# RKWin93/E2E-MAPPO-for-MT-FJSP

Hardware: AMD Instinct MI355X
Metric: env-steps/sec (batched J6M6E2) (higher is better)
Workload: dtype f64 (environment) / f32 (encoder: f32 storage and accumulation; 128x128 products on the 16-bit matrix cores from split f32 operands, f32-accurate: DESIGN.md §4)

## Files before the change

__graft_entry__.py:

```python
#!/usr/bin/env python3
import os
import sys

ROOT = os.path.dirname(os.path.abspath(__file__))
if ROOT not in sys.path:
    sys.path.insert(0, ROOT)


def build() -> None:
    from importlib import import_module
    import mtfjsp_amd
    _build = import_module("e2e-mappo-for-mt-fjsp_amd._build")
    lib = _build.build(force=True, verbose=True)
    capi = import_module("e2e-mappo-for-mt-fjsp_amd.capi")
    capi.lib()
    print("variant:", _build.build_variant("funcs", ["-DMTFJSP_BODY_FUNCS=3"]))
    from oracle import env_oracle
    print("oracle:", env_oracle.build(force=True))
    print("built", lib)


def smoke() -> None:
    import numpy as np
    import torch
    from importlib import import_module
    import mtfjsp_amd
    assert torch.cuda.is_available(), "smoke() needs cuda:0"
    batch_env = import_module("e2e-mappo-for-mt-fjsp_amd.batch_env")
    inst = import_module("e2e-mappo-for-mt-fjsp_amd.instances")
    from oracle.env_oracle import OracleBatch
    J, M, E, B = 6, 6, 2, 8
    T = J * M
    t, p, tt, edge = inst.generate_instances(B, J, M, E, seed=0)
    import random
    random.seed(0)
    w3 = inst.random_weights(B)
    env = batch_env.DeviceBatchEnv(J, M, E, B, obs_dtype="f64")
    env.load_instances(t, p, tt, edge=edge)
    env.scaler_init()
    env.reset(w3)
    orc = OracleBatch(t, p, tt, edge)
    orc.scaler_init()
    orc.reset(w3)
    a = torch.zeros(B, dtype=torch.int32, device=env.device); m = torch.zeros_like(a); j = torch.zeros_like(a)
    for s in range(T):
        env.random_actions(7, s, a, m, j)
        env.step(a, m)
        info, raw, _ = orc.step(a.cpu().numpy(), m.cpu().numpy())
        cand, mask = orc.job_mask_update(j.cpu().numpy())
        o = orc.observe()
        assert np.array_equal(env.info.cpu().numpy(), info), f"step {s}: rewards differ"
        assert np.array_equal(env.tasks_fea.cpu().numpy(), o["tfea"]), f"step {s}: tasks_fea differ"
        assert np.array_equal(env.dense_adj().cpu().numpy(), o["adj"]), f"step {s}: adj differ"
        assert np.array_equal(env.m_fea2.cpu().numpy(), o["mfea2"])
        assert np.array_equal(env.candidate.cpu().numpy(), cand) and np.array_equal(env.job_mask.cpu().numpy(), mask)
    assert bool(env.info[:, 1].all())
    _smoke_encoder()
    print("smoke OK: HIP env == oracle on", B, "instances x", T, "steps")


def _smoke_encoder() -> None:
    try:
        from importlib import import_module
        enc = import_module("e2e-mappo-for-mt-fjsp_amd.encoder")
    except ImportError:
        return
    if hasattr(enc, "smoke"):
        enc.smoke()


if __name__ == "__main__":
    cmd = sys.argv[1] if len(sys.argv) > 1 else "build"
    {"build": build, "smoke": smoke}[cmd]()
```

e2e-mappo-for-mt-fjsp_amd/_build.py:

```python
import os
import shutil
import subprocess

PKG = os.path.dirname(os.path.abspath(__file__))
CSRC = os.path.join(PKG, "csrc")
LIB = os.path.join(PKG, "libmtfjsp.so")
SOURCES = ["mtfjsp_env.hip", "mtfjsp_encoder.hip", "mtfjsp_gin_res.hip", "mtfjsp_pdr.hip", "mtfjsp_lookahead.hip", "mtfjsp_beam.hip", "mtfjsp_group.hip", "mtfjsp_hostgen.cpp"]
FLAGS = ["--offload-arch=gfx950", "-O3", "-ffp-contract=off", "-fPIC", "-std=c++17", "-Wall"]
SOURCE_FLAGS = {"mtfjsp_env.hip": ["-mllvm", "-amdgpu-sched-strategy=max-ilp"], "mtfjsp_gin_res.hip": ["-mllvm", "-amdgpu-sched-strategy=max-ilp"]}
if os.environ.get("MTFJSP_NO_SOURCE_FLAGS"):
    SOURCE_FLAGS = {}
if os.environ.get("MTFJSP_SOURCE_FLAGS_JSON"):
    import json
    SOURCE_FLAGS = json.loads(os.environ["MTFJSP_SOURCE_FLAGS_JSON"])


def hipcc():
    for c in (os.environ.get("HIPCC"), shutil.which("hipcc"), "/opt/rocm/bin/hipcc"):
        if c and os.path.exists(c):
            return c
    raise RuntimeError("hipcc not found")


def needs_build():
    if not os.path.exists(LIB):
        return True
    t = os.path.getmtime(LIB)
    deps = [os.path.join(CSRC, s) for s in SOURCES if os.path.exists(os.path.join(CSRC, s))]
    deps.append(os.path.join(PKG, "..", "include", "mtfjsp.h"))
    deps += [os.path.join(CSRC, f) for f in os.listdir(CSRC) if f.endswith((".h", ".hpp"))]
    return any(os.path.getmtime(d) > t for d in deps)


def _compile_link(out, extra_flags, verbose=False):
    import concurrent.futures
    import tempfile
    srcs = [s for s in SOURCES if os.path.exists(os.path.join(CSRC, s))]
    with tempfile.TemporaryDirectory(prefix="mtfjsp_build_") as tmp:
        def one(src):
            obj = os.path.join(tmp, src + ".o")
            cmd = [hipcc()] + FLAGS + SOURCE_FLAGS.get(src, []) + list(extra_flags) + ["-c", os.path.join(CSRC, src), "-o", obj]
            if verbose:
                print(" ".join(cmd))
            subprocess.check_call(cmd)
            return obj
        with concurrent.futures.ThreadPoolExecutor(len(srcs)) as ex:
            objs = list(ex.map(one, srcs))
        cmd = [hipcc(), "--offload-arch=gfx950", "-shared", "-fPIC"] + objs + ["-o", out]
        if verbose:
            print(" ".join(cmd))
        subprocess.check_call(cmd)
    return out


def build(force=False, verbose=False):
    if not force and not needs_build():
        return LIB
    return _compile_link(LIB, [], verbose)


def build_variant(tag, extra_flags, verbose=False):
    out = os.path.join(PKG, f"libmtfjsp_{tag}.so")
    srcs = [os.path.join(CSRC, s) for s in SOURCES]
    import hashlib
    hsh = hashlib.sha256(" ".join(FLAGS + list(extra_flags) + [repr(sorted(SOURCE_FLAGS.items()))]).encode())
    for d in sorted(srcs + [os.path.join(CSRC, f) for f in os.listdir(CSRC) if f.endswith((".h", ".hpp"))] + [os.path.join(PKG, "..", "include", "mtfjsp.h")]):
        hsh.update(open(d, "rb").read())
    stamp = out + ".srchash"
    if os.path.exists(out) and os.path.exists(stamp) and open(stamp).read() == hsh.hexdigest() and not os.environ.get("MTFJSP_REBUILD_VARIANTS"):
        return out
    _compile_link(out, extra_flags, verbose)
    with open(stamp, "w") as f:
        f.write(hsh.hexdigest())
    return out


if __name__ == "__main__":
    print(build(force=True, verbose=True))
```

e2e-mappo-for-mt-fjsp_amd/csrc/mtfjsp_gin_resident.h:

```cpp
#ifndef GR_KERNEL
#ifndef MTFJSP_GIN_RESIDENT_H
#define MTFJSP_GIN_RESIDENT_H
#include <type_traits>
#include <utility>
#include "mtfjsp_gin_res_select.h"

#ifndef GR_ABL
#define GR_ABL 0
#endif
#ifndef GR_NRES
#define GR_NRES 16
#endif
#ifndef GR_VRES
#define GR_VRES 1
#endif
#define GR_RING 6
#define GR_NBAR 6
#ifndef GR_GRP
#define GR_GRP 2
#endif
#ifndef GR_LOOK
#define GR_LOOK 2
#endif
#define GR_ROWB 272
#define GR_PLANE (32 * GR_ROWB)
#define GR_TILE (2 * GR_PLANE)
#define GR_MAXWARM 10
#ifndef GR_FX_DROP
#define GR_FX_DROP 1
#endif
#ifndef GR_FX_TAIL
#define GR_FX_TAIL 1
#endif
#ifndef GR_FX_SETUP
#define GR_FX_SETUP 1
#endif
struct GrShapeAny { static constexpr bool FIXED = false; static constexpr int T = 0, J = 0, IPC = 0; };
template <int T_, int J_, int IPC_> struct GrShapeFixed {
    static constexpr bool FIXED = true; static constexpr int T = T_, J = J_, IPC = IPC_;
    static_assert(T_ >= GR_MINT && T_ <= GR_MAXT && IPC_ * T_ == GR_ROWS && IPC_ * J_ <= GR_MAXCAND && (IPC_ * 128) % 256 == 0, "fixed shape: full 576-row workgroups");
};
typedef GrShapeFixed<GIN_RES_FX_T, GIN_RES_FX_J, GIN_RES_FX_IPC> GrShapeHeadline;
constexpr int gr_left_at(int T, int h, int rt)
{
    int left = ((16 * h) / T + 1) * T - 16 * h;
    for (int i = 0; i < rt; i++) { left -= 32; if (left <= 0) left += T; if (left <= 0) left += T; }
    return left;
}
constexpr int gr_max_chunks(int T)
{
    int m = 0;
    for (int i = 0; i < 16; i++) { const int r0 = i * T, c = ((r0 + T - 1) >> 4) - (r0 >> 4) + 1; m = c > m ? c : m; }
    return m;
}

#ifndef GR_MIX
#define GR_MIX 2
#endif
#ifndef GR_SETTLE
#define GR_SETTLE 1
#endif
#ifndef GR_FOLD_DPP
#define GR_FOLD_DPP 1
#endif
#ifndef GR_STAT_ASM
#define GR_STAT_ASM 0
#endif
#ifndef GR_PK
#define GR_PK 1
#endif
typedef float f32x16 __attribute__((ext_vector_type(16)));
typedef _Float16 gr_h8 __attribute__((ext_vector_type(8)));
typedef _Float16 gr_h2 __attribute__((ext_vector_type(2)));

struct GinResArgs {
    int B, T, J, ipc;
    const void *tfea; int feat_f64;
    const int *ell_col; const float *ell_val;
    const void *Wx32[6];
    float wsinv[6];
    const float *gamma[6], *beta[6];
    unsigned long long *stats;
    unsigned long long *stats_next;
    int wexp[6];
    int ffrac[6];
    unsigned long long *bar;
    unsigned long long epoch;
    unsigned *fail;
    unsigned *range_flag;
    const int *candidate;
    float *pooled;
    float *cand_feat;
    float *h_nodes;
    float *zspill;
    double inv_rows;
    int barrier_only;
    unsigned expect_extra;
    unsigned long long *stamps;
    const void *warm[GR_MAXWARM];
    unsigned warm_lines[GR_MAXWARM];
    int nwarm;
};
#define GR_STATS_PART (6 * 8 * HD * 2)
#define GR_STATS_SET GR_STATS_PART
#ifdef GR_STAMP
#define GR_STAMP_AT(i) do { if (tid == 0 && A.stamps) { A.stamps[(size_t)blockIdx.x * 64 + (i)] = __builtin_amdgcn_s_memrealtime(); \
                                                         if ((i) <= 30) A.stamps[(size_t)blockIdx.x * 64 + 33 + (i)] = __builtin_amdgcn_s_memtime(); } } while (0)
#else
#define GR_STAMP_AT(i) do { } while (0)
#endif

#define GR_OFF_PLANES 0
#define GR_OFF_RING (2 * GR_TILE)
#define GR_RING_BYTES ((2 * GR_LOOK - 2) * GR_TILE > GR_RING * 32 * HD * 4 ? (2 * GR_LOOK - 2) * GR_TILE : GR_RING * 32 * HD * 4)
#define GR_OFF_ELLC (GR_OFF_RING + GR_RING_BYTES)
#define GR_OFF_ELLV0 (GR_OFF_ELLC + GR_ROWS * 4)
#define GR_OFF_ELLV1 (GR_OFF_ELLV0 + GR_ROWS * 4)
#define GR_OFF_BN (GR_OFF_ELLV1 + GR_ROWS * 4)
#define GR_OFF_CAND (GR_OFF_BN + 2 * HD * 4)
// ... 280 lines not shown
        if (GR_ABL & 4) return;
#pragma unroll
        for (int i = 0; i < 8; i++) stat2(i, a[2 * i], a[2 * i + 1]);
    };
    auto split2x4 = [&](f32x2 v01, f32x2 v23, uint2 &p0, uint2 &p1) __attribute__((always_inline)) {
        const gr_h2 a = __builtin_convertvector(v01, gr_h2), b = __builtin_convertvector(v23, gr_h2);
#if GR_MIX == 2
        const gr_h2 c = gr_rem16(v01, a), d = gr_rem16(v23, b);
#else
        const f32x2 r01 = gr_rem2(v01, a), r23 = gr_rem2(v23, b);
        const gr_h2 c = __builtin_convertvector(r01, gr_h2), d = __builtin_convertvector(r23, gr_h2);
#endif
        p0 = make_uint2(__builtin_bit_cast(unsigned, a), __builtin_bit_cast(unsigned, b));
        p1 = make_uint2(__builtin_bit_cast(unsigned, c), __builtin_bit_cast(unsigned, d));
    };
    auto stats_tile = [&](auto Tc) __attribute__((always_inline)) {
        constexpr int RT = decltype(Tc)::value;
        stats_all(GR_TILEVAL(RT));
    };
    auto fold_stats = [&]() __attribute__((always_inline)) {
        float *red = s_ring;
        float *mine = red + (wave * 64 + lane) * 36;
#pragma unroll
        for (int j = 0; j < 4; j++) {
            *reinterpret_cast<float4 *>(mine + 4 * j) = make_float4(ts[2 * j][0], ts[2 * j][1], ts[2 * j + 1][0], ts[2 * j + 1][1]);
            *reinterpret_cast<float4 *>(mine + 16 + 4 * j) = make_float4(tq[2 * j][0], tq[2 * j][1], tq[2 * j + 1][0], tq[2 * j + 1][1]);
        }
#pragma unroll
        for (int i = 0; i < 8; i++) { ts[i] = f32x2{0.f, 0.f}; tq[i] = f32x2{0.f, 0.f}; }
        LDS_BARRIER();
        const int col = tid >> 1, kind = tid & 1, cw = col & 31;
        const float *src = red + ((col >> 5) * 64 + 32 * ((cw >> 2) & 1)) * 36 + 4 * (cw >> 3) + (cw & 3) + 16 * kind;
        float s0 = 0.f, s1 = 0.f, s2 = 0.f, s3 = 0.f;
#pragma unroll
        for (int i = 0; i < 32; i += 4) { s0 += src[i * 36]; s1 += src[(i + 1) * 36]; s2 += src[(i + 2) * 36]; s3 += src[(i + 3) * 36]; }
        return (s0 + s1) + (s2 + s3);
    };
    auto fold_stats_dpp = [&]() __attribute__((always_inline)) {
        const bool b4 = (lane & 16) != 0, b3 = (lane & 8) != 0, b2 = (lane & 4) != 0, b1 = (lane & 2) != 0, b0 = (lane & 1) != 0;
        auto dpp = [&](float x, auto Ctrl) __attribute__((always_inline)) {
            return __builtin_bit_cast(float, __builtin_amdgcn_update_dpp(0, __builtin_bit_cast(int, x), decltype(Ctrl)::value, 0xF, 0xF, true));
        };
        float v16[16];
#pragma unroll
        for (int c = 0; c < 16; c++) {
            const float a = ts[c >> 1][c & 1], q_ = tq[c >> 1][c & 1];
            v16[c] = (b4 ? q_ : a) + __shfl_xor(b4 ? a : q_, 16);
        }
#pragma unroll
        for (int i = 0; i < 8; i++) { ts[i] = f32x2{0.f, 0.f}; tq[i] = f32x2{0.f, 0.f}; }
        float v8[8];
#pragma unroll
        for (int c = 0; c < 8; c++) v8[c] = (b3 ? v16[c + 8] : v16[c]) + dpp(b3 ? v16[c] : v16[c + 8], std::integral_constant<int, 0x140>{});
        float v4[4];
#pragma unroll
        for (int c = 0; c < 4; c++) v4[c] = (b2 ? v8[c + 4] : v8[c]) + dpp(b2 ? v8[c] : v8[c + 4], std::integral_constant<int, 0x141>{});
        float v2[2];
#pragma unroll
        for (int c = 0; c < 2; c++) v2[c] = (b1 ? v4[c + 2] : v4[c]) + dpp(b1 ? v4[c] : v4[c + 2], std::integral_constant<int, 0x4E>{});
        return (b0 ? v2[1] : v2[0]) + dpp(b0 ? v2[0] : v2[1], std::integral_constant<int, 0xB1>{});
    };
    unsigned char *const pl0 = s_planes, *const pl1 = s_planes + GR_TILE, *const plr = reinterpret_cast<unsigned char *>(s_ring);
    auto plane_buf = [&](int i) __attribute__((always_inline)) { return i == 0 ? pl0 : i == 1 ? pl1 : plr + (i - 2) * GR_TILE; };
    auto produce_quarter = [&](auto Tc, auto Gc, unsigned char *pbuf) __attribute__((always_inline)) {
        constexpr int rt = decltype(Tc)::value, g = decltype(Gc)::value;
        unsigned char *dst = pbuf + n * GR_ROWB + (32 * wave + 8 * g + 4 * h) * 2;
        const float *bn = bn_of(rt);
        const float4 s4 = *reinterpret_cast<const float4 *>(bn + 32 * wave + 8 * g + 4 * h);
        const float4 h4 = *reinterpret_cast<const float4 *>(bn + HD + 32 * wave + 8 * g + 4 * h);
        const f32x16 &a = GR_TILEVAL(rt);
        uint2 p0, p1;
        split2x4(f32x2{bn_relu_ss(a[4 * g], s4.x, h4.x), bn_relu_ss(a[4 * g + 1], s4.y, h4.y)},
                 f32x2{bn_relu_ss(a[4 * g + 2], s4.z, h4.z), bn_relu_ss(a[4 * g + 3], s4.w, h4.w)}, p0, p1);
        *reinterpret_cast<uint2 *>(dst) = p0;
        *reinterpret_cast<uint2 *>(dst + GR_PLANE) = p1;
    };
    auto produce_tile = [&](auto Tc, unsigned char *pbuf) __attribute__((always_inline)) {
        gr_static_for<4>([&](auto Gc) __attribute__((always_inline)) { produce_quarter(Tc, Gc, pbuf); });
        __builtin_amdgcn_sched_barrier(0);
    };
    const unsigned char *xa0 = s_planes + n * GR_ROWB + 16 * h;
#define GR_FENCE() __builtin_amdgcn_sched_barrier(0)
#define GR_PIN_V() do { } while (0)
    auto consume_tile = [&](auto Tc) __attribute__((always_inline)) {
        constexpr int RT = decltype(Tc)::value;
        constexpr int PT = RT + GR_LOOK;
        constexpr bool NEXT = (PT < GR_NT) && !(GR_ABL & 1);
        constexpr bool STATS = RT > 0 && (GR_VRES || RT - 1 < GR_NRES) && !(GR_ABL & 4);
        const unsigned char *xa = plane_buf(RT % (2 * GR_LOOK)) + n * GR_ROWB + 16 * h;
        unsigned char *pnext = plane_buf(PT % (2 * GR_LOOK));
        const float *bn = bn_of(PT);
        gr_h8 xf[2][2];
#pragma unroll
        for (int p = 0; p < 2; p++) xf[0][p] = *reinterpret_cast<const gr_h8 *>(xa + p * GR_PLANE);
        float4 s4 = make_float4(0.f, 0.f, 0.f, 0.f), h4 = s4;
        if constexpr (NEXT) {
            s4 = *reinterpret_cast<const float4 *>(bn + 32 * wave + 4 * h);
            h4 = *reinterpret_cast<const float4 *>(bn + HD + 32 * wave + 4 * h);
        }
        constexpr bool VT = GR_VRES && RT >= GR_NRES;
        f32x16 atmp;
        f32x16 &a = RT < GR_NRES ? acc[RT < GR_NRES ? RT : 0] : VT ? zs[RT >= GR_NRES ? (RT - GR_NRES) & 1 : 0] : atmp;
        if constexpr (RT + GR_LOOK + 1 >= GR_NRES && RT + GR_LOOK + 1 < GR_NT) zload(std::integral_constant<int, RT + GR_LOOK + 1 - GR_NRES>{});
        gr_static_for<4>([&](auto Pc) __attribute__((always_inline)) {
            constexpr int g = decltype(Pc)::value;
            const gr_h8 *x0 = xf[0], *x1 = xf[1];
            f32x2 v01 = {0.f, 0.f}, v23 = {0.f, 0.f}, e01 = v01, e23 = v01;
            gr_h2 p01 = {0, 0}, p23 = p01, q01 = p01, q23 = p01;
            unsigned char *dst = pnext + n * GR_ROWB + (32 * wave + 8 * g + 4 * h) * 2;
            const f32x16 &nx = GR_TILEVAL(PT < GR_NT ? PT : RT);
            const f32x16 &pv = GR_TILEVAL(RT > 0 ? RT - 1 : 0);
            auto M = [&](int ks, int wp, int xp) __attribute__((always_inline)) {
                if (GR_ABL & 2) return;
                if constexpr (VT) mfma_v(a, wf[wp][ks], (ks & 1) ? x1[xp] : x0[xp], ks == 0 && wp == 0 && xp == 1);
                else if (ks == 0 && wp == 0 && xp == 1)
                    a = __builtin_amdgcn_mfma_f32_32x32x16_f16(wf[wp][ks], x0[xp], f32x16{0.f, 0.f, 0.f, 0.f, 0.f, 0.f, 0.f, 0.f, 0.f, 0.f, 0.f, 0.f, 0.f, 0.f, 0.f, 0.f}, 0, 0, 0);
                else a = __builtin_amdgcn_mfma_f32_32x32x16_f16(wf[wp][ks], (ks & 1) ? x1[xp] : x0[xp], a, 0, 0, 0);
            };
            M(2 * g, 0, 1);
            xf[1][0] = *reinterpret_cast<const gr_h8 *>(xa + 32 * (2 * g + 1));
            if constexpr (NEXT) { v01 = gr_fma2(f32x2{nx[4 * g], nx[4 * g + 1]}, f32x2{s4.x, s4.y}, f32x2{h4.x, h4.y});
                                  v23 = gr_fma2(f32x2{nx[4 * g + 2], nx[4 * g + 3]}, f32x2{s4.z, s4.w}, f32x2{h4.z, h4.w}); }
            GR_FENCE();
            M(2 * g, 1, 0);
            xf[1][1] = *reinterpret_cast<const gr_h8 *>(xa + GR_PLANE + 32 * (2 * g + 1));
            if constexpr (NEXT) { v01 = __builtin_elementwise_max(v01, f32x2{0.f, 0.f}); v23 = __builtin_elementwise_max(v23, f32x2{0.f, 0.f}); }
            GR_FENCE();
            M(2 * g, 0, 0);
            if constexpr (NEXT) { p01 = __builtin_convertvector(v01, gr_h2); p23 = __builtin_convertvector(v23, gr_h2); }
            if constexpr (NEXT && g < 3) s4 = *reinterpret_cast<const float4 *>(bn + 32 * wave + 8 * (g + 1) + 4 * h);
            GR_FENCE();
            M(2 * g + 1, 0, 1);
            if constexpr (g < 3) xf[0][0] = *reinterpret_cast<const gr_h8 *>(xa + 32 * (2 * g + 2));
            if constexpr (NEXT && !GR_MIX) { e01 = __builtin_convertvector(p01, f32x2); e23 = __builtin_convertvector(p23, f32x2); }
            if constexpr (NEXT && g < 3) h4 = *reinterpret_cast<const float4 *>(bn + HD + 32 * wave + 8 * (g + 1) + 4 * h);
            GR_FENCE();
            M(2 * g + 1, 1, 0);
            if constexpr (g < 3) xf[0][1] = *reinterpret_cast<const gr_h8 *>(xa + GR_PLANE + 32 * (2 * g + 2));
            if constexpr (NEXT) { if constexpr (GR_MIX == 2) { q01 = gr_rem16(v01, p01); q23 = gr_rem16(v23, p23); }
                                  else if constexpr (GR_MIX == 1) { v01 = gr_rem2(v01, p01); v23 = gr_rem2(v23, p23); } else { v01 = gr_sub2(v01, e01); v23 = gr_sub2(v23, e23); }
                                  if (!(GR_ABL & 8)) *reinterpret_cast<uint2 *>(dst) = make_uint2(__builtin_bit_cast(unsigned, p01), __builtin_bit_cast(unsigned, p23));
                                  if constexpr (GR_MIX != 2) { q01 = __builtin_convertvector(v01, gr_h2); q23 = __builtin_convertvector(v23, gr_h2); } }
            GR_FENCE();
            M(2 * g + 1, 0, 0);
            if constexpr (NEXT) { if (!(GR_ABL & 8)) *reinterpret_cast<uint2 *>(dst + GR_PLANE) = make_uint2(__builtin_bit_cast(unsigned, q01), __builtin_bit_cast(unsigned, q23));
                                  else asm volatile("" :: "v"(p01), "v"(p23), "v"(q01), "v"(q23)); }
            if constexpr (STATS) { stat2(2 * g, pv[4 * g], pv[4 * g + 1]); stat2(2 * g + 1, pv[4 * g + 2], pv[4 * g + 3]); }
            GR_FENCE();
        });
        if constexpr (RT >= GR_NRES && !GR_VRES) {
            stats_all(a);
            zstore(std::integral_constant<int, RT - GR_NRES>{}, a);
            GR_FENCE();
        }
        if constexpr (!VT && GR_SETTLE) { asm volatile("s_nop 1"); GR_FENCE(); }
    };
    auto consume_tile0 = [&](auto Tc) __attribute__((always_inline)) {
        constexpr int RT = decltype(Tc)::value;
        const unsigned char *xa = xa0 + 32 * (RT & 7);
        bf16x8 x[3];
#pragma unroll
        for (int p = 0; p < 3; p++) x[p] = *reinterpret_cast<const bf16x8 *>(xa + p * GR_PLANE);
        f32x16 a = {0.f, 0.f, 0.f, 0.f, 0.f, 0.f, 0.f, 0.f, 0.f, 0.f, 0.f, 0.f, 0.f, 0.f, 0.f, 0.f};
        a = __builtin_amdgcn_mfma_f32_32x32x16_bf16(w0f[0], x[2], a, 0, 0, 0);
        a = __builtin_amdgcn_mfma_f32_32x32x16_bf16(w0f[2], x[0], a, 0, 0, 0);
        a = __builtin_amdgcn_mfma_f32_32x32x16_bf16(w0f[1], x[1], a, 0, 0, 0);
        a = __builtin_amdgcn_mfma_f32_32x32x16_bf16(w0f[0], x[1], a, 0, 0, 0);
        a = __builtin_amdgcn_mfma_f32_32x32x16_bf16(w0f[1], x[0], a, 0, 0, 0);
        a = __builtin_amdgcn_mfma_f32_32x32x16_bf16(w0f[0], x[0], a, 0, 0, 0);
        if constexpr (RT < GR_NRES) acc[RT] = a;
        else if constexpr (GR_VRES) zs[(RT - GR_NRES) & 1] = a;
        else {
            stats_all(a);
            zstore(std::integral_constant<int, RT - GR_NRES>{}, a);
        }
        if constexpr (RT > 0 && (GR_VRES || RT - 1 < GR_NRES)) stats_tile(std::integral_constant<int, RT - 1>{});
        __builtin_amdgcn_sched_barrier(0);
    };
    float *s_wtab = s_ring + 1024 + 4 * (2 * 32 * 36);
    static_assert(!(GR_FX_SETUP && GR_FOLD_DPP) || (1024 + 4 * (2 * 32 * 36)) * 4 >= (2 * GR_LOOK - 2) * GR_TILE, "s_wtab lies past the plane buffers in the ring area");
    unsigned warm_word = 0;
    int slot[GR_NT];
    auto final_setup_a = [&]() __attribute__((always_inline)) {
        int tid_s = tid;
        if constexpr (FXS) asm volatile("" : "+v"(tid_s));
        for (int i = tid_s; i < 17 * 16; i += 256) s_wtab[i] = (i & 15) < (i >> 4) ? 1.0f : 0.0f;
        if (A.nwarm > 0) {
            unsigned l = (blockIdx.x >> 3) * 256u + (unsigned)tid_s;
            const unsigned char *wp = reinterpret_cast<const unsigned char *>(A.warm[0]);
            bool found = false;
            for (int w = 0; w < A.nwarm; w++) {
                const unsigned nl = A.warm_lines[w];
                if (!found && l < nl) { wp = reinterpret_cast<const unsigned char *>(A.warm[w]) + (size_t)l * 128; found = true; }
                if (!found) l -= nl;
            }
            warm_word = *reinterpret_cast<const unsigned *>(wp);
        }
    };
    auto final_setup_b = [&]() __attribute__((always_inline)) {
#ifndef GR_KEEP_MASKS
        asm volatile("" : "+v"(n_l));
#endif
#pragma unroll
        for (int rt = 0; rt < GR_NT; rt++) slot[rt] = (GR_ABL & 32) ? -1 : s_rowcand[rt * 32 + n_l];
    };
    auto layer_boundary = [&](auto Kc) __attribute__((always_inline)) {
        constexpr int k = decltype(Kc)::value;
        GR_STAMP_AT(4 + 4 * k);
        if constexpr (GR_VRES && GR_NT > GR_NRES) {
            asm volatile("s_nop 15\n\ts_nop 15" ::: "memory");
            stats_all(zs[(GR_NT - 1 - GR_NRES) & 1]);
        }
#if GR_FOLD_DPP
        (void)fold_stats;
        const float colsum = fold_stats_dpp();
        int lane_b = lane;
        if constexpr (FXS && k == 5) asm volatile("" : "+v"(lane_b));
        const int n_b = lane_b & 31, h_b = lane_b >> 5;
        const int kind = n_b >> 4, scol = 32 * wave + 8 * ((n_b & 15) >> 2) + 4 * h_b + (n_b & 3);
        constexpr int PAIR = 16;
#else
        const float colsum = fold_stats();
        const int kind = tid & 1, scol = tid >> 1;
        constexpr int PAIR = 1;
#endif
        const int sidx = 2 * scol + kind;
        if (k == 1) GR_STAMP_AT(2);
        const unsigned grp = blockIdx.x & 7u;
        {
            float x = colsum;
            if (!(__builtin_fabsf(x) * (kind ? A.wsinv[k] * A.wsinv[k] : A.wsinv[k]) < __builtin_ldexpf(1.0f, 51 - A.ffrac[k]))) {
                if (A.range_flag && !timed_out) __hip_atomic_store(A.range_flag, 1u, __ATOMIC_RELAXED, __HIP_MEMORY_SCOPE_SYSTEM);
// ... 97 lines not shown
#ifndef GR_KEEP_MASKS
        if constexpr (FXD) asm volatile("" : "+v"(n_l));
        else asm volatile("" : "+s"(nrows_l), "+v"(n_l));
#endif
        if constexpr (layer != 3) {
            gr_static_for<GR_LOOK>([&](auto Ic) __attribute__((always_inline)) { produce_tile(Ic, plane_buf(decltype(Ic)::value)); });
            LDS_BARRIER();
            unsigned *cnt = s_cnt + (layer - 1) * (GR_NT / GR_GRP);
            gr_static_for<GR_NT>([&](auto Tc) __attribute__((always_inline)) {
                constexpr int RT = decltype(Tc)::value;
                constexpr int step = RT / GR_GRP, back = GR_LOOK / GR_GRP;
                if constexpr (GR_LOOK > GR_GRP && RT % GR_GRP == 0 && step >= back) {
                    while (__builtin_amdgcn_readfirstlane(__hip_atomic_load(&cnt[step - back], __ATOMIC_RELAXED, __HIP_MEMORY_SCOPE_WORKGROUP)) < 4u)
                        __builtin_amdgcn_s_sleep(1);
                    asm volatile("" ::: "memory");
                    __builtin_amdgcn_sched_barrier(0);
                }
                consume_tile(Tc);
                GR_PIN_V();
                if constexpr (RT % GR_GRP == GR_GRP - 1) {
                    if constexpr (GR_LOOK > GR_GRP) {
                        asm volatile("" ::: "memory");
                        if (lane == 0) __hip_atomic_fetch_add(&cnt[step], 1u, __ATOMIC_RELAXED, __HIP_MEMORY_SCOPE_WORKGROUP);
                    } else LDS_BARRIER();
                }
                __builtin_amdgcn_sched_barrier(0);
            });
            if constexpr (GR_LOOK > GR_GRP) LDS_BARRIER();
            static_assert(GR_NT % GR_GRP == 0 && GR_GRP >= 1 && (GR_LOOK == GR_GRP || GR_LOOK == 2 * GR_GRP) && GR_LOOK <= GR_NRES, "tile groups");
        } else {
            auto write_h = [&](auto Tc) __attribute__((always_inline)) {
                constexpr int rt = decltype(Tc)::value;
                float *base = s_ring + ((rt % GR_RING) * 32 + n) * HD;
                gr_static_for<4>([&](auto Gc) __attribute__((always_inline)) {
                    constexpr int g = decltype(Gc)::value;
                    const float *bn = bn_of(rt);
                    const float4 s4 = *reinterpret_cast<const float4 *>(bn + 32 * wave + 8 * g + 4 * h);
                    const float4 h4 = *reinterpret_cast<const float4 *>(bn + HD + 32 * wave + 8 * g + 4 * h);
                    const f32x16 &a = GR_TILEVAL(rt);
                    const int ch = (8 * wave + 2 * g + h) ^ (n & 7);
                    *reinterpret_cast<float4 *>(base + 4 * ch) = make_float4(bn_relu_ss(a[4 * g], s4.x, h4.x), bn_relu_ss(a[4 * g + 1], s4.y, h4.y),
                                                                             bn_relu_ss(a[4 * g + 2], s4.z, h4.z), bn_relu_ss(a[4 * g + 3], s4.w, h4.w));
                });
                __builtin_amdgcn_sched_barrier(0);
            };
            auto ring_row = [&](int R) __attribute__((always_inline)) {
                const int t = R >> 5;
                return ((t - GR_RING * ((t * 43) >> 8)) * 32 + (R & 31)) * HD;
            };
            struct AggRow { const float *po, *px, *py; float w0, w1, inv; int s0, s1, s2; };
            auto agg_row = [&](int RT) __attribute__((always_inline)) {
                AggRow r;
                const int row = RT * 32 + n_l;
                const unsigned cp = s_ellc[row];
                const unsigned r0 = cp & 0xffffu, r1 = cp >> 16;
                r.w0 = s_ellv0[row]; r.w1 = s_ellv1[row];
                const int deg = 1 + (r0 != 0xffffu) + (r1 != 0xffffu);
                r.inv = deg == 1 ? 1.0f : deg == 2 ? 0.5f : (1.0f / 3.0f);
                const int n0 = r0 != 0xffffu ? (int)r0 : row, n1 = r1 != 0xffffu ? (int)r1 : row;
                r.po = s_ring + ((RT % GR_RING) * 32 + n) * HD; r.px = s_ring + ring_row(n0); r.py = s_ring + ring_row(n1);
                r.s0 = n & 7; r.s1 = n0 & 7; r.s2 = n1 & 7;
                return r;
            };
            auto agg_quarter_standalone = [&](const AggRow &r, int g, unsigned char *dst) __attribute__((always_inline)) {
                const int chl = 8 * wave + 2 * g + h;
                const float4 o = *reinterpret_cast<const float4 *>(r.po + 4 * (chl ^ r.s0));
                const float4 x = *reinterpret_cast<const float4 *>(r.px + 4 * (chl ^ r.s1));
                const float4 y = *reinterpret_cast<const float4 *>(r.py + 4 * (chl ^ r.s2));
                const f32x2 W0 = {r.w0, r.w0}, W1 = {r.w1, r.w1}, IV = {r.inv, r.inv};
                const f32x2 v01 = gr_mul2(gr_fma2(W1, f32x2{y.x, y.y}, gr_fma2(W0, f32x2{x.x, x.y}, f32x2{o.x, o.y})), IV);
                const f32x2 v23 = gr_mul2(gr_fma2(W1, f32x2{y.z, y.w}, gr_fma2(W0, f32x2{x.z, x.w}, f32x2{o.z, o.w})), IV);
                uint2 p0, p1;
                split2x4(v01, v23, p0, p1);
                *reinterpret_cast<uint2 *>(dst + 16 * g) = p0;
                *reinterpret_cast<uint2 *>(dst + 16 * g + GR_PLANE) = p1;
            };
            auto consume_agg = [&](auto Tc) __attribute__((always_inline)) {
                constexpr int RT = decltype(Tc)::value;
                constexpr bool NEXT = RT + 1 < GR_NT && !(GR_ABL & 1);
                constexpr bool WH = RT + 4 < GR_NT && !(GR_ABL & 1);
                constexpr int WT = WH ? RT + 4 : RT;
                constexpr bool STATS = RT > 0 && (GR_VRES || RT - 1 < GR_NRES) && !(GR_ABL & 4);
                constexpr bool VT = GR_VRES && RT >= GR_NRES;
                const unsigned char *xa = xa0 + (RT & 1) * GR_TILE;
                gr_h8 xf[2][2];
#pragma unroll
                for (int p = 0; p < 2; p++) xf[0][p] = *reinterpret_cast<const gr_h8 *>(xa + p * GR_PLANE);
                AggRow r = agg_row(NEXT ? RT + 1 : RT);
                unsigned char *dst = s_planes + ((RT + 1) & 1) * GR_TILE + n * GR_ROWB + (32 * wave + 4 * h) * 2;
                const float *bnw = bn_of(WT);
                float *hbase = s_ring + ((WT % GR_RING) * 32 + n) * HD;
                float4 s4 = make_float4(0.f, 0.f, 0.f, 0.f), h4 = s4;
                if constexpr (WH) {
                    s4 = *reinterpret_cast<const float4 *>(bnw + 32 * wave + 4 * h);
                    h4 = *reinterpret_cast<const float4 *>(bnw + HD + 32 * wave + 4 * h);
                }
                f32x16 atmp;
                f32x16 &a = RT < GR_NRES ? acc[RT < GR_NRES ? RT : 0] : VT ? zs[RT >= GR_NRES ? (RT - GR_NRES) & 1 : 0] : atmp;
                if constexpr (RT + 6 >= GR_NRES && RT + 6 < GR_NT) zload(std::integral_constant<int, RT + 6 - GR_NRES>{});
                gr_static_for<4>([&](auto Pc) __attribute__((always_inline)) {
                    constexpr int g = decltype(Pc)::value;
                    const gr_h8 *x0 = xf[0], *x1 = xf[1];
                    const f32x16 &wv = GR_TILEVAL(WT);
                    const f32x16 &pv = GR_TILEVAL(RT > 0 ? RT - 1 : 0);
                    const int chl = 8 * wave + 2 * g + h;
                    float4 o = make_float4(0.f, 0.f, 0.f, 0.f), x = o, y = o;
                    f32x2 v01 = {0.f, 0.f}, v23 = v01, e01 = v01, e23 = v01, u01 = v01, u23 = v01;
                    gr_h2 p01 = {0, 0}, p23 = p01, q01 = p01, q23 = p01;
                    const f32x2 W0 = {r.w0, r.w0}, W1 = {r.w1, r.w1}, IV = {r.inv, r.inv};
                    auto M = [&](int ks, int wp, int xp) __attribute__((always_inline)) {
                        if (!(GR_ABL & 2)) {
                            if constexpr (VT) mfma_v(a, wf[wp][ks], (ks & 1) ? x1[xp] : x0[xp], g == 0 && ks == 0 && wp == 0 && xp == 1);
                            else if (g == 0 && ks == 0 && wp == 0 && xp == 1)
                                a = __builtin_amdgcn_mfma_f32_32x32x16_f16(wf[wp][ks], x0[xp], f32x16{0.f, 0.f, 0.f, 0.f, 0.f, 0.f, 0.f, 0.f, 0.f, 0.f, 0.f, 0.f, 0.f, 0.f, 0.f, 0.f}, 0, 0, 0);
                            else a = __builtin_amdgcn_mfma_f32_32x32x16_f16(wf[wp][ks], (ks & 1) ? x1[xp] : x0[xp], a, 0, 0, 0);
                        }
                    };
                    M(2 * g, 0, 1);
                    xf[1][0] = *reinterpret_cast<const gr_h8 *>(xa + 32 * (2 * g + 1));
                    if constexpr (NEXT) { o = *reinterpret_cast<const float4 *>(r.po + 4 * (chl ^ r.s0)); x = *reinterpret_cast<const float4 *>(r.px + 4 * (chl ^ r.s1));
                                          y = *reinterpret_cast<const float4 *>(r.py + 4 * (chl ^ r.s2)); }
                    if constexpr (STATS) { stat2(2 * g, pv[4 * g], pv[4 * g + 1]); stat2(2 * g + 1, pv[4 * g + 2], pv[4 * g + 3]); }
                    GR_FENCE();
                    M(2 * g, 1, 0);
                    xf[1][1] = *reinterpret_cast<const gr_h8 *>(xa + GR_PLANE + 32 * (2 * g + 1));
                    if constexpr (WH) { u01 = __builtin_elementwise_max(gr_fma2(f32x2{wv[4 * g], wv[4 * g + 1]}, f32x2{s4.x, s4.y}, f32x2{h4.x, h4.y}), f32x2{0.f, 0.f});
                                        u23 = __builtin_elementwise_max(gr_fma2(f32x2{wv[4 * g + 2], wv[4 * g + 3]}, f32x2{s4.z, s4.w}, f32x2{h4.z, h4.w}), f32x2{0.f, 0.f}); }
                    GR_FENCE();
                    M(2 * g, 0, 0);
                    if constexpr (WH) *reinterpret_cast<float4 *>(hbase + 4 * (chl ^ (n & 7))) = make_float4(u01[0], u01[1], u23[0], u23[1]);
                    if constexpr (NEXT) { v01 = gr_fma2(W0, f32x2{x.x, x.y}, f32x2{o.x, o.y}); v23 = gr_fma2(W0, f32x2{x.z, x.w}, f32x2{o.z, o.w}); }
                    if constexpr (WH && g < 3) s4 = *reinterpret_cast<const float4 *>(bnw + 32 * wave + 8 * (g + 1) + 4 * h);
                    GR_FENCE();
                    M(2 * g + 1, 0, 1);
                    if constexpr (g < 3) xf[0][0] = *reinterpret_cast<const gr_h8 *>(xa + 32 * (2 * g + 2));
                    if constexpr (NEXT) { v01 = gr_fma2(W1, f32x2{y.x, y.y}, v01); v23 = gr_fma2(W1, f32x2{y.z, y.w}, v23); }
                    if constexpr (WH && g < 3) h4 = *reinterpret_cast<const float4 *>(bnw + HD + 32 * wave + 8 * (g + 1) + 4 * h);
                    GR_FENCE();
                    M(2 * g + 1, 1, 0);
                    if constexpr (g < 3) xf[0][1] = *reinterpret_cast<const gr_h8 *>(xa + GR_PLANE + 32 * (2 * g + 2));
                    if constexpr (NEXT) { v01 = gr_mul2(v01, IV); v23 = gr_mul2(v23, IV); p01 = __builtin_convertvector(v01, gr_h2); p23 = __builtin_convertvector(v23, gr_h2);
                                          if constexpr (!GR_MIX) { e01 = __builtin_convertvector(p01, f32x2); e23 = __builtin_convertvector(p23, f32x2); } }
                    GR_FENCE();
                    M(2 * g + 1, 0, 0);
                    if constexpr (NEXT) { if constexpr (GR_MIX == 2) { q01 = gr_rem16(v01, p01); q23 = gr_rem16(v23, p23); }
                                          else { if constexpr (GR_MIX) { v01 = gr_rem2(v01, p01); v23 = gr_rem2(v23, p23); } else { v01 = gr_sub2(v01, e01); v23 = gr_sub2(v23, e23); } q01 = __builtin_convertvector(v01, gr_h2); q23 = __builtin_convertvector(v23, gr_h2); }
                                          *reinterpret_cast<uint2 *>(dst + 16 * g) = make_uint2(__builtin_bit_cast(unsigned, p01), __builtin_bit_cast(unsigned, p23));
                                          *reinterpret_cast<uint2 *>(dst + 16 * g + GR_PLANE) = make_uint2(__builtin_bit_cast(unsigned, q01), __builtin_bit_cast(unsigned, q23)); }
                    GR_FENCE();
                });
                if constexpr (RT >= GR_NRES && !GR_VRES) {
                    stats_all(a);
                    zstore(std::integral_constant<int, RT - GR_NRES>{}, a);
                    GR_FENCE();
                }
                if constexpr (!VT && GR_SETTLE) { asm volatile("s_nop 1"); GR_FENCE(); }
            };
            write_h(std::integral_constant<int, 0>{}); write_h(std::integral_constant<int, 1>{}); write_h(std::integral_constant<int, 2>{});
            write_h(std::integral_constant<int, 3>{});
            LDS_BARRIER();
            {
                const AggRow r = agg_row(0);
                unsigned char *dst = s_planes + n * GR_ROWB + (32 * wave + 4 * h) * 2;
#pragma unroll
                for (int g = 0; g < 4; g++) agg_quarter_standalone(r, g, dst);
            }
            LDS_BARRIER();
            __builtin_amdgcn_sched_barrier(0);
            gr_static_for<GR_NT>([&](auto Tc) __attribute__((always_inline)) {
                consume_agg(Tc);
                LDS_BARRIER();
                __builtin_amdgcn_sched_barrier(0);
            });
        }
        layer_boundary(std::integral_constant<int, layer>{});
    });

    GR_STAMP_AT(30);
    {
        int lane_f = lane;
        asm volatile("" : "+v"(lane_f));
        const int n_f = lane_f & 31, h_f = lane_f >> 5;
        float *s_part = reinterpret_cast<float *>(s_planes);
        static_assert(2 * GR_NT * 2 * HD * 4 <= 2 * GR_TILE + 4096, "partial pool sums: plane buffers + 4 KB");
        float *tb = s_ring + 1024 + wave * (2 * 32 * 36);
        if constexpr (!FXS) final_setup_a();
        float4 S[4], Hs[4];
#pragma unroll
        for (int g = 0; g < 4; g++) {
            S[g] = *reinterpret_cast<const float4 *>(s_bn + 32 * wave + 8 * g + 4 * h_f);
            Hs[g] = *reinterpret_cast<const float4 *>(s_bn + HD + 32 * wave + 8 * g + 4 * h_f);
        }
        if constexpr (GR_NT - GR_NRES >= 1) zload(std::integral_constant<int, 0>{});
        if constexpr (GR_NT - GR_NRES >= 2) zload(std::integral_constant<int, 1>{});
        const int c = lane_f & 31;
        int left = ((16 * h_f) / T + 1) * T - 16 * h_f;
        auto left_at = [&](auto Rc) __attribute__((always_inline)) {
            constexpr int rt = decltype(Rc)::value;
            constexpr int FT = FXD ? SH::T : GR_MINT;
            if constexpr (FXD) return h_f ? gr_left_at(FT, 1, rt) : gr_left_at(FT, 0, rt);
            else return left;
        };
        if constexpr (!FXS) { final_setup_b(); LDS_BARRIER(); }
        unsigned char *const cbase = reinterpret_cast<unsigned char *>(A.cand_feat + (size_t)inst0 * Jn * HD);
        const unsigned coff = (unsigned)(32 * wave + 4 * h_f) * 4u;
        GR_STAMP_AT(28);
        float x[16];
        float4 w0, w1, w2, w3;
        auto pool_load = [&](auto Rc) __attribute__((always_inline)) {
            constexpr int rt = decltype(Rc)::value;
            const int lf = left_at(Rc);
            const float *rb = tb + (rt & 1) * (32 * 36) + (16 * h_f) * 36 + c;
#pragma unroll
            for (int i = 0; i < 16; i++) x[i] = rb[i * 36];
            const float4 *wt = reinterpret_cast<const float4 *>(s_wtab + (lf < 16 ? lf : 16) * 16);
            w0 = wt[0]; w1 = wt[1]; w2 = wt[2]; w3 = wt[3];
        };
        auto pool_math = [&](auto Rc) __attribute__((always_inline)) {
            constexpr int rt = decltype(Rc)::value;
            const int lf = left_at(Rc);
            f32x2 sa2 = gr_fma2(f32x2{x[0], x[1]}, f32x2{w0.x, w0.y}, f32x2{0.f, 0.f});
            sa2 = gr_fma2(f32x2{x[2], x[3]}, f32x2{w0.z, w0.w}, sa2);
            sa2 = gr_fma2(f32x2{x[4], x[5]}, f32x2{w1.x, w1.y}, sa2);
            sa2 = gr_fma2(f32x2{x[6], x[7]}, f32x2{w1.z, w1.w}, sa2);
            sa2 = gr_fma2(f32x2{x[8], x[9]}, f32x2{w2.x, w2.y}, sa2);
            sa2 = gr_fma2(f32x2{x[10], x[11]}, f32x2{w2.z, w2.w}, sa2);
            sa2 = gr_fma2(f32x2{x[12], x[13]}, f32x2{w3.x, w3.y}, sa2);
            sa2 = gr_fma2(f32x2{x[14], x[15]}, f32x2{w3.z, w3.w}, sa2);
            const f32x2 t2 = gr_add2(gr_add2(gr_add2(f32x2{x[0], x[1]}, f32x2{x[2], x[3]}), gr_add2(f32x2{x[4], x[5]}, f32x2{x[6], x[7]})),
                                     gr_add2(gr_add2(f32x2{x[8], x[9]}, f32x2{x[10], x[11]}), gr_add2(f32x2{x[12], x[13]}, f32x2{x[14], x[15]})));
            const float tot = t2[0] + t2[1];
            const float sa = sa2[0] + sa2[1];
            float *pp = s_part + ((2 * rt + h_f) * 2) * HD + 32 * wave + c;
// ... 98 lines not shown
```

Before: 21.60 million.

## Prefetch next tile's operands and BN params across tile seams in resident GIN

Inside the resident GIN encoder's tile loops, the first operand fragments and batch-norm scale/shift of the next tile are now loaded during the last group of the current tile and carried across the seam in registers. The order of operand-plane loads is also changed so that each fragment is fetched one step earlier than the MFMA that consumes it. The aim is to hide LDS load latency at the start of each tile, at the cost of extra live registers. A SEAM0 build variant that turns this off is added for comparison.

```diff
diff --git a/__graft_entry__.py b/__graft_entry__.py
--- a/__graft_entry__.py
+++ b/__graft_entry__.py
@@ -15,6 +15,7 @@
     capi = import_module("e2e-mappo-for-mt-fjsp_amd.capi")
     capi.lib()
     print("variant:", _build.build_variant("funcs", ["-DMTFJSP_BODY_FUNCS=3"]))
+    print("variant:", _build.build_variant(*_build.SEAM0))
     from oracle import env_oracle
     print("oracle:", env_oracle.build(force=True))
     print("built", lib)
diff --git a/e2e-mappo-for-mt-fjsp_amd/_build.py b/e2e-mappo-for-mt-fjsp_amd/_build.py
--- a/e2e-mappo-for-mt-fjsp_amd/_build.py
+++ b/e2e-mappo-for-mt-fjsp_amd/_build.py
@@ -59,20 +59,32 @@
     return _compile_link(LIB, [], verbose)
 
 
-def build_variant(tag, extra_flags, verbose=False):
-    out = os.path.join(PKG, f"libmtfjsp_{tag}.so")
+def variant_hash(extra_flags):
+    import hashlib
     srcs = [os.path.join(CSRC, s) for s in SOURCES]
-    import hashlib
     hsh = hashlib.sha256(" ".join(FLAGS + list(extra_flags) + [repr(sorted(SOURCE_FLAGS.items()))]).encode())
     for d in sorted(srcs + [os.path.join(CSRC, f) for f in os.listdir(CSRC) if f.endswith((".h", ".hpp"))] + [os.path.join(PKG, "..", "include", "mtfjsp.h")]):
         hsh.update(open(d, "rb").read())
-    stamp = out + ".srchash"
-    if os.path.exists(out) and os.path.exists(stamp) and open(stamp).read() == hsh.hexdigest() and not os.environ.get("MTFJSP_REBUILD_VARIANTS"):
+    return hsh.hexdigest()
+
+
+def variant_paths(tag):
+    out = os.path.join(PKG, f"libmtfjsp_{tag}.so")
+    return out, out + ".srchash"
+
+
+def build_variant(tag, extra_flags, verbose=False):
+    out, stamp = variant_paths(tag)
+    digest = variant_hash(extra_flags)
+    if os.path.exists(out) and os.path.exists(stamp) and open(stamp).read() == digest and not os.environ.get("MTFJSP_REBUILD_VARIANTS"):
         return out
     _compile_link(out, extra_flags, verbose)
     with open(stamp, "w") as f:
-        f.write(hsh.hexdigest())
+        f.write(digest)
     return out
+
+
+SEAM0 = ("seam0", ["-DGR_SEAM=0"])
 
 
 if __name__ == "__main__":
diff --git a/e2e-mappo-for-mt-fjsp_amd/csrc/mtfjsp_gin_resident.h b/e2e-mappo-for-mt-fjsp_amd/csrc/mtfjsp_gin_resident.h
--- a/e2e-mappo-for-mt-fjsp_amd/csrc/mtfjsp_gin_resident.h
+++ b/e2e-mappo-for-mt-fjsp_amd/csrc/mtfjsp_gin_resident.h
@@ -35,6 +35,19 @@
 #ifndef GR_FX_SETUP
 #define GR_FX_SETUP 1
 #endif
+#ifndef GR_SEAM
+#define GR_SEAM 1
+#endif
+#ifndef GR_SEAM_XF
+#define GR_SEAM_XF 1
+#endif
+#ifndef GR_SEAM_BN
+#define GR_SEAM_BN 1
+#endif
+#ifndef GR_SEAM_AGG
+#define GR_SEAM_AGG 1
+#endif
+#define GR_SEAM_ON(item) (GR_SEAM && (item))
 struct GrShapeAny { static constexpr bool FIXED = false; static constexpr int T = 0, J = 0, IPC = 0; };
 template <int T_, int J_, int IPC_> struct GrShapeFixed {
     static constexpr bool FIXED = true; static constexpr int T = T_, J = J_, IPC = IPC_;
@@ -481,6 +494,8 @@
     const unsigned char *xa0 = s_planes + n * GR_ROWB + 16 * h;
 #define GR_FENCE() __builtin_amdgcn_sched_barrier(0)
 #define GR_PIN_V() do { } while (0)
+    gr_h8 xfc[3];
+    float4 s4c, h4c;
     auto consume_tile = [&](auto Tc) __attribute__((always_inline)) {
         constexpr int RT = decltype(Tc)::value;
         constexpr int PT = RT + GR_LOOK;
@@ -489,11 +504,25 @@
         const unsigned char *xa = plane_buf(RT % (2 * GR_LOOK)) + n * GR_ROWB + 16 * h;
         unsigned char *pnext = plane_buf(PT % (2 * GR_LOOK));
         const float *bn = bn_of(PT);
+        constexpr bool XF_OUT = GR_SEAM_ON(GR_SEAM_XF) && GR_LOOK == GR_GRP && RT + 1 < GR_NT && RT % GR_GRP != GR_GRP - 1;
+        constexpr bool XF_IN = GR_SEAM_ON(GR_SEAM_XF) && GR_LOOK == GR_GRP && RT > 0 && (RT - 1) % GR_GRP != GR_GRP - 1;
+        constexpr bool BN_OUT = GR_SEAM_ON(GR_SEAM_BN) && NEXT && PT + 1 < GR_NT, BN_IN = GR_SEAM_ON(GR_SEAM_BN) && NEXT && RT > 0;
+        constexpr bool ORD = GR_SEAM_ON(GR_SEAM_XF);
+        const unsigned char *xan = plane_buf((RT + 1) % (2 * GR_LOOK)) + n * GR_ROWB + 16 * h;
+        const float *bnn = bn_of(PT + 1);
         gr_h8 xf[2][2];
 #pragma unroll
-        for (int p = 0; p < 2; p++) xf[0][p] = *reinterpret_cast<const gr_h8 *>(xa + p * GR_PLANE);
+        for (int p = 0; p < 2; p++) {
+            if constexpr (XF_IN) xf[0][p] = xfc[p];
+            else xf[0][ORD ? 1 - p : p] = *reinterpret_cast<const gr_h8 *>(xa + (ORD ? 1 - p : p) * GR_PLANE);
+        }
+        if constexpr (ORD) {
+            if constexpr (XF_IN) xf[1][1] = xfc[2];
+            else xf[1][1] = *reinterpret_cast<const gr_h8 *>(xa + GR_PLANE + 32);
+        }
         float4 s4 = make_float4(0.f, 0.f, 0.f, 0.f), h4 = s4;
-        if constexpr (NEXT) {
+        if constexpr (BN_IN) { s4 = s4c; h4 = h4c; }
+        else if constexpr (NEXT) {
             s4 = *reinterpret_cast<const float4 *>(bn + 32 * wave + 4 * h);
             h4 = *reinterpret_cast<const float4 *>(bn + HD + 32 * wave + 4 * h);
         }
@@ -522,20 +551,27 @@
                                   v23 = gr_fma2(f32x2{nx[4 * g + 2], nx[4 * g + 3]}, f32x2{s4.z, s4.w}, f32x2{h4.z, h4.w}); }
             GR_FENCE();
             M(2 * g, 1, 0);
-            xf[1][1] = *reinterpret_cast<const gr_h8 *>(xa + GR_PLANE + 32 * (2 * g + 1));
+            if constexpr (!ORD) xf[1][1] = *reinterpret_cast<const gr_h8 *>(xa + GR_PLANE + 32 * (2 * g + 1));
+            else if constexpr (g < 3) xf[0][1] = *reinterpret_cast<const gr_h8 *>(xa + GR_PLANE + 32 * (2 * g + 2));
+            else if constexpr (XF_OUT) xf[0][1] = *reinterpret_cast<const gr_h8 *>(xan + GR_PLANE);
             if constexpr (NEXT) { v01 = __builtin_elementwise_max(v01, f32x2{0.f, 0.f}); v23 = __builtin_elementwise_max(v23, f32x2{0.f, 0.f}); }
             GR_FENCE();
             M(2 * g, 0, 0);
             if constexpr (NEXT) { p01 = __builtin_convertvector(v01, gr_h2); p23 = __builtin_convertvector(v23, gr_h2); }
             if constexpr (NEXT && g < 3) s4 = *reinterpret_cast<const float4 *>(bn + 32 * wave + 8 * (g + 1) + 4 * h);
+            if constexpr (BN_OUT && g == 3) s4 = *reinterpret_cast<const float4 *>(bnn + 32 * wave + 4 * h);
             GR_FENCE();
             M(2 * g + 1, 0, 1);
             if constexpr (g < 3) xf[0][0] = *reinterpret_cast<const gr_h8 *>(xa + 32 * (2 * g + 2));
+            if constexpr (XF_OUT && g == 3) xf[0][0] = *reinterpret_cast<const gr_h8 *>(xan);
             if constexpr (NEXT && !GR_MIX) { e01 = __builtin_convertvector(p01, f32x2); e23 = __builtin_convertvector(p23, f32x2); }
             if constexpr (NEXT && g < 3) h4 = *reinterpret_cast<const float4 *>(bn + HD + 32 * wave + 8 * (g + 1) + 4 * h);
+            if constexpr (BN_OUT && g == 3) h4 = *reinterpret_cast<const float4 *>(bnn + HD + 32 * wave + 4 * h);
             GR_FENCE();
             M(2 * g + 1, 1, 0);
-            if constexpr (g < 3) xf[0][1] = *reinterpret_cast<const gr_h8 *>(xa + GR_PLANE + 32 * (2 * g + 2));
+            if constexpr (!ORD) { if constexpr (g < 3) xf[0][1] = *reinterpret_cast<const gr_h8 *>(xa + GR_PLANE + 32 * (2 * g + 2)); }
+            else if constexpr (g < 3) xf[1][1] = *reinterpret_cast<const gr_h8 *>(xa + GR_PLANE + 32 * (2 * g + 3));
+            else if constexpr (XF_OUT) xf[1][1] = *reinterpret_cast<const gr_h8 *>(xan + GR_PLANE + 32);
             if constexpr (NEXT) { if constexpr (GR_MIX == 2) { q01 = gr_rem16(v01, p01); q23 = gr_rem16(v23, p23); }
                                   else if constexpr (GR_MIX == 1) { v01 = gr_rem2(v01, p01); v23 = gr_rem2(v23, p23); } else { v01 = gr_sub2(v01, e01); v23 = gr_sub2(v23, e23); }
                                   if (!(GR_ABL & 8)) *reinterpret_cast<uint2 *>(dst) = make_uint2(__builtin_bit_cast(unsigned, p01), __builtin_bit_cast(unsigned, p23));
@@ -547,6 +583,8 @@
             if constexpr (STATS) { stat2(2 * g, pv[4 * g], pv[4 * g + 1]); stat2(2 * g + 1, pv[4 * g + 2], pv[4 * g + 3]); }
             GR_FENCE();
         });
+        if constexpr (XF_OUT) { xfc[0] = xf[0][0]; xfc[1] = xf[0][1]; xfc[2] = xf[1][1]; }
+        if constexpr (BN_OUT) { s4c = s4; h4c = h4; }
         if constexpr (RT >= GR_NRES && !GR_VRES) {
             stats_all(a);
             zstore(std::integral_constant<int, RT - GR_NRES>{}, a);
@@ -810,16 +848,21 @@
                 constexpr int WT = WH ? RT + 4 : RT;
                 constexpr bool STATS = RT > 0 && (GR_VRES || RT - 1 < GR_NRES) && !(GR_ABL & 4);
                 constexpr bool VT = GR_VRES && RT >= GR_NRES;
+                constexpr bool ORD = GR_SEAM_ON(GR_SEAM_AGG);
                 const unsigned char *xa = xa0 + (RT & 1) * GR_TILE;
                 gr_h8 xf[2][2];
 #pragma unroll
-                for (int p = 0; p < 2; p++) xf[0][p] = *reinterpret_cast<const gr_h8 *>(xa + p * GR_PLANE);
+                for (int p = 0; p < 2; p++) xf[0][ORD ? 1 - p : p] = *reinterpret_cast<const gr_h8 *>(xa + (ORD ? 1 - p : p) * GR_PLANE);
+                if constexpr (ORD) xf[1][1] = *reinterpret_cast<const gr_h8 *>(xa + GR_PLANE + 32);
                 AggRow r = agg_row(NEXT ? RT + 1 : RT);
                 unsigned char *dst = s_planes + ((RT + 1) & 1) * GR_TILE + n * GR_ROWB + (32 * wave + 4 * h) * 2;
                 const float *bnw = bn_of(WT);
                 float *hbase = s_ring + ((WT % GR_RING) * 32 + n) * HD;
+                constexpr bool BN_OUT = GR_SEAM_ON(GR_SEAM_AGG) && WH && RT + 5 < GR_NT, BN_IN = GR_SEAM_ON(GR_SEAM_AGG) && WH && RT > 0;
+                const float *bnn = bn_of(WT + 1);
                 float4 s4 = make_float4(0.f, 0.f, 0.f, 0.f), h4 = s4;
-                if constexpr (WH) {
+                if constexpr (BN_IN) { s4 = s4c; h4 = h4c; }
+                else if constexpr (WH) {
                     s4 = *reinterpret_cast<const float4 *>(bnw + 32 * wave + 4 * h);
                     h4 = *reinterpret_cast<const float4 *>(bnw + HD + 32 * wave + 4 * h);
                 }
@@ -851,7 +894,8 @@
                     if constexpr (STATS) { stat2(2 * g, pv[4 * g], pv[4 * g + 1]); stat2(2 * g + 1, pv[4 * g + 2], pv[4 * g + 3]); }
                     GR_FENCE();
                     M(2 * g, 1, 0);
-                    xf[1][1] = *reinterpret_cast<const gr_h8 *>(xa + GR_PLANE + 32 * (2 * g + 1));
+                    if constexpr (!ORD) xf[1][1] = *reinterpret_cast<const gr_h8 *>(xa + GR_PLANE + 32 * (2 * g + 1));
+                    else if constexpr (g < 3) xf[0][1] = *reinterpret_cast<const gr_h8 *>(xa + GR_PLANE + 32 * (2 * g + 2));
                     if constexpr (WH) { u01 = __builtin_elementwise_max(gr_fma2(f32x2{wv[4 * g], wv[4 * g + 1]}, f32x2{s4.x, s4.y}, f32x2{h4.x, h4.y}), f32x2{0.f, 0.f});
                                         u23 = __builtin_elementwise_max(gr_fma2(f32x2{wv[4 * g + 2], wv[4 * g + 3]}, f32x2{s4.z, s4.w}, f32x2{h4.z, h4.w}), f32x2{0.f, 0.f}); }
                     GR_FENCE();
@@ -859,14 +903,17 @@
                     if constexpr (WH) *reinterpret_cast<float4 *>(hbase + 4 * (chl ^ (n & 7))) = make_float4(u01[0], u01[1], u23[0], u23[1]);
                     if constexpr (NEXT) { v01 = gr_fma2(W0, f32x2{x.x, x.y}, f32x2{o.x, o.y}); v23 = gr_fma2(W0, f32x2{x.z, x.w}, f32x2{o.z, o.w}); }
                     if constexpr (WH && g < 3) s4 = *reinterpret_cast<const float4 *>(bnw + 32 * wave + 8 * (g + 1) + 4 * h);
+                    if constexpr (BN_OUT && g == 3) s4 = *reinterpret_cast<const float4 *>(bnn + 32 * wave + 4 * h);
                     GR_FENCE();
                     M(2 * g + 1, 0, 1);
                     if constexpr (g < 3) xf[0][0] = *reinterpret_cast<const gr_h8 *>(xa + 32 * (2 * g + 2));
                     if constexpr (NEXT) { v01 = gr_fma2(W1, f32x2{y.x, y.y}, v01); v23 = gr_fma2(W1, f32x2{y.z, y.w}, v23); }
                     if constexpr (WH && g < 3) h4 = *reinterpret_cast<const float4 *>(bnw + HD + 32 * wave + 8 * (g + 1) + 4 * h);
+                    if constexpr (BN_OUT && g == 3) h4 = *reinterpret_cast<const float4 *>(bnn + HD + 32 * wave + 4 * h);
                     GR_FENCE();
                     M(2 * g + 1, 1, 0);
-                    if constexpr (g < 3) xf[0][1] = *reinterpret_cast<const gr_h8 *>(xa + GR_PLANE + 32 * (2 * g + 2));
+                    if constexpr (!ORD) { if constexpr (g < 3) xf[0][1] = *reinterpret_cast<const gr_h8 *>(xa + GR_PLANE + 32 * (2 * g + 2)); }
+                    else if constexpr (g < 3) xf[1][1] = *reinterpret_cast<const gr_h8 *>(xa + GR_PLANE + 32 * (2 * g + 3));
                     if constexpr (NEXT) { v01 = gr_mul2(v01, IV); v23 = gr_mul2(v23, IV); p01 = __builtin_convertvector(v01, gr_h2); p23 = __builtin_convertvector(v23, gr_h2);
                                           if constexpr (!GR_MIX) { e01 = __builtin_convertvector(p01, f32x2); e23 = __builtin_convertvector(p23, f32x2); } }
                     GR_FENCE();
@@ -877,6 +924,7 @@
                                           *reinterpret_cast<uint2 *>(dst + 16 * g + GR_PLANE) = make_uint2(__builtin_bit_cast(unsigned, q01), __builtin_bit_cast(unsigned, q23)); }
                     GR_FENCE();
                 });
+                if constexpr (BN_OUT) { s4c = s4; h4c = h4; }
                 if constexpr (RT >= GR_NRES && !GR_VRES) {
                     stats_all(a);
                     zstore(std::integral_constant<int, RT - GR_NRES>{}, a);
```

Result: no change. 21.75 million, median of 5 (+0.7%).
